# DrQuestion/monica

Measured on AMD Instinct MI355X. Metric: reads/sec classified, higher is better.
Workload: dtype u32/u64 integer; int16 pairs in the alignment kernels (int32 / int8 in the long-call and literal ones); float32 islands: overlap ratio, MAPQ

## Files before the change

monica_amd/csrc/k_fill.hip:

```cpp
#include "device.h"

namespace mnc {

constexpr int FILL_NEG = -(1 << 28);
constexpr int FILL_WIN = 16;
constexpr int FILL_MIN_BAND = 8;
constexpr int FILL_CIG_MAX = 384;
constexpr size_t FILL_P_SLOT = (size_t)(2 * FILL_MAX_LEN + FILL_WIN) * 64;

__device__ __forceinline__ void fill_order()
{
	__builtin_amdgcn_fence(__ATOMIC_SEQ_CST, "wavefront");
	asm volatile("" ::: "memory");
}
__device__ __forceinline__ void fill_order_mem()
{
	__builtin_amdgcn_fence(__ATOMIC_SEQ_CST, "workgroup");
	asm volatile("" ::: "memory");
}

__device__ __forceinline__ int fill_nt4(uint8_t c)
{
	switch (c) {
	case 'A': case 'a': return 0;
	case 'C': case 'c': return 1;
	case 'G': case 'g': return 2;
	case 'T': case 't': case 'U': case 'u': return 3;
	default: return 4;
	}
}

__device__ __forceinline__ int fill_qcode(const Batch &B, bool acgt, int64_t roff, const uint8_t *read, int rlen, int rev, int pq)
{
	const int p = rev ? rlen - 1 - pq : pq;
	if (acgt) {
		const int64_t g = roff + p;
		const int c = (int)(B.packed[g >> 4] >> (30 - 2 * (int)(g & 15)) & 3u);
		return rev ? 3 - c : c;
	}
	const int c = fill_nt4(read[p]);
	return rev ? (c < 4 ? 3 - c : 4) : c;
}

__device__ __forceinline__ uint32_t fill_qcodes16(const Batch &B, int64_t roff, int rlen, int rev, int pq)
{
	int64_t g0 = rev ? roff + rlen - 16 - pq : roff + pq;
	int skip = 0;
	if (g0 < 0) skip = (int)-g0, g0 = 0;
	const uint32_t hi = B.packed[g0 >> 4], lo = B.packed[(g0 >> 4) + 1];
	const uint32_t sh2 = 2 * (uint32_t)(g0 & 15);
	uint32_t f = sh2 ? __builtin_amdgcn_alignbit(hi, lo, 32 - sh2) : hi;
	if (rev) return ~f >> (2 * skip);
	f = __builtin_bitreverse32(f);
	return (f & 0x55555555u) << 1 | (f >> 1 & 0x55555555u);
}

__host__ __device__ __forceinline__ int fill_gap(int l, int q, int e, int q2, int e2)
{
	const int g1 = q + e * l, g2 = q2 + e2 * l;
	return g1 < g2 ? g1 : g2;
}

__host__ __device__ __forceinline__ void fill_band(int n, int m, int cells, int &b, int &kmin, int &kmax)
{
	const int d = n - m, ad = d < 0 ? -d : d;
	b = (2 * cells - 2 - ad) / 2;
	kmin = (d < 0 ? d : 0) - b;
	if (kmin & 1) --kmin;
	kmax = kmin + 2 * cells - 1;
}

__host__ __device__ __forceinline__ int dp_band_bound(int n, int m, int kmin, int kmax, int a, int q, int e, int q2, int e2)
{
	const int d = n - m;
	int U = FILL_NEG;
	{
		const int D0 = kmax + 1, I0 = kmax + 1 - d, left = n - D0;
		if (left >= 0 && m - I0 >= 0) {
			const int u = a * left - fill_gap(D0, q, e, q2, e2) - fill_gap(I0, q, e, q2, e2);
			U = U > u ? U : u;
		}
	}
	{
// ... 189 lines not shown
			fill_order();
		}
		bool walk = leader && ok && !to_next && !to_fb;
		if (walk) {
			int mcols = 0, g2 = 0, kd = 0, kbest = 0;
			for (int k = 0; k < n_c; ++k) {
				const uint32_t op = s_cg[sg][k] & 0xf;
				const int len = (int)(s_cg[sg][k] >> 4);
				if (op == 0) mcols += len, kd = kd - a * len > 0 ? kd - a * len : 0;
				else g2 += fill_gap(len, q, e, q2, e2), kd += q + e * len, kbest = kbest > kd ? kbest : kd;
			}
			const int lost = a * mcols - S - g2;
			const int neg = kbest + lost;
			if (neg <= (B.zdrop_inv < B.zdrop ? B.zdrop_inv : B.zdrop)) walk = false;
		}
		if (walk) {
			int score = 0, mx = INT32_MIN, max_i = -1, max_j = -1, i = 0, j = 0, max_zdrop = 0;
			for (int k = n_c - 1; k >= 0; --k) {
				const uint32_t op = s_cg[sg][k] & 0xf;
				const int len = (int)(s_cg[sg][k] >> 4);
				if (op == 0) {
					for (int l = 0; l < len; ++l) {
						const int ct = s_t[sg][i + l], cq = s_q[sg][j + l];
						score += (ct == 4 || cq == 4) ? scN : ct == cq ? a : bmis;
						if (score < mx) {
							const int li = i + l - max_i, lj = j + l - max_j;
							const int z = mx - score - (li > lj ? li - lj : lj - li) * e;
							max_zdrop = max_zdrop > z ? max_zdrop : z;
						} else mx = score, max_i = i + l, max_j = j + l;
					}
					i += len, j += len;
				} else {
					score -= q + e * len;
					if (op == 1) j += len; else i += len;
					if (score < mx) {
						const int li = i - max_i, lj = j - max_j;
						const int z = mx - score - (li > lj ? li - lj : lj - li) * e;
						max_zdrop = max_zdrop > z ? max_zdrop : z;
					} else mx = score, max_i = i, max_j = j;
				}
			}
			if (max_zdrop > (B.zdrop_inv < B.zdrop ? B.zdrop_inv : B.zdrop)) to_fb = true;
		}
		const bool s_next = __shfl((int)to_next, lead) != 0, s_fb = __shfl((int)to_fb, lead) != 0;
		const int s_nc = __shfl(n_c, lead);
		if (has && (s_next || s_fb)) {
			if (leader) {
				const bool literal = s_fb || next_list == fb_list;
				if (literal && (B.segs[si].flag & SEG_NEEDS_BIG_WS)) { const unsigned long long k = atomicAdd(&B.dp_ctr[56], 1ULL); B.bigfb_list[k] = (int32_t)si; }
				else if (literal) { const unsigned long long k = atomicAdd(&B.dp_ctr[ctr_fb], 1ULL); fb_list[k] = (int32_t)si; }
				else { const unsigned long long k = atomicAdd(&B.dp_ctr[ctr_next], 1ULL); next_list[k] = (int32_t)si; }
			}
		} else if (has) {
			unsigned long long off = 0;
			if (leader) off = atomicAdd(&B.dp_ctr[1], (unsigned long long)s_nc);
			off = (unsigned long long)__shfl((long long)off, lead);
			int wrote = s_nc;
			if ((long long)(off + s_nc) > B.cig_seg_cap) {
				if (leader) atomicMax(&B.dp_ctr[4], 2ULL);
				wrote = 0;
			} else for (int k = L; k < s_nc; k += LANES) B.cig_seg[off + k] = s_cg[sg][s_nc - 1 - k];
			if (leader) {
				Seg *o = B.segs + si;
				o->n_cigar = wrote, o->zdropped = 0, o->zdrop_code = 0;
				o->max = 0, o->max_t = -1, o->max_q = -1, o->score = S, o->reach_end = 0, o->mqe_t = -1;
				o->cig_off = (int64_t)off;
			}
		}
		fill_order_mem();
	}
}

typedef short pk_s16 __attribute__((ext_vector_type(2)));
typedef unsigned short pk_u16 __attribute__((ext_vector_type(2)));
__device__ __forceinline__ uint32_t pk_adds(uint32_t x, uint32_t y) { return __builtin_bit_cast(uint32_t, __builtin_elementwise_add_sat(__builtin_bit_cast(pk_s16, x), __builtin_bit_cast(pk_s16, y))); }
__device__ __forceinline__ uint32_t pk_subs(uint32_t x, uint32_t y) { return __builtin_bit_cast(uint32_t, __builtin_elementwise_sub_sat(__builtin_bit_cast(pk_s16, x), __builtin_bit_cast(pk_s16, y))); }
__device__ __forceinline__ uint32_t pk_maxs(uint32_t x, uint32_t y) { return __builtin_bit_cast(uint32_t, __builtin_elementwise_max(__builtin_bit_cast(pk_s16, x), __builtin_bit_cast(pk_s16, y))); }
__device__ __forceinline__ uint32_t pk_subsu(uint32_t x, uint32_t y) { return __builtin_bit_cast(uint32_t, __builtin_elementwise_sub_sat(__builtin_bit_cast(pk_u16, x), __builtin_bit_cast(pk_u16, y))); }
__device__ __forceinline__ uint32_t pk_madu(uint32_t x, uint32_t y, uint32_t z) { return __builtin_bit_cast(uint32_t, (pk_u16)(__builtin_bit_cast(pk_u16, x) * __builtin_bit_cast(pk_u16, y) + __builtin_bit_cast(pk_u16, z))); }
__device__ __forceinline__ uint32_t pk_rep(int v) { return ((uint32_t)v & 0xffffu) * 0x10001u; }
__device__ __forceinline__ uint32_t pk_bfi(uint32_t mask, uint32_t x, uint32_t y) { return (x & mask) | (y & ~mask); }

constexpr uint32_t PK_NEG = 0x80008000u;
__device__ __forceinline__ uint32_t fillp_opened(uint32_t x)
{
	const uint32_t d = (x & 1u) ^ 1u, c = (x >> 1 & 1u) ^ d, b = (x >> 2 & 1u) ^ 1u ^ c ^ d, a = (x >> 3 & 1u) ^ b ^ c ^ d;
	return a << 3 | b << 2 | c << 1 | d;
}
constexpr uint32_t PK_TAG_H = 0x000f000fu, PK_TAG_E = 0x00070007u, PK_TAG_F = 0x00030003u, PK_TAG_E2 = 0x00010001u;
struct PkConst { uint32_t kmatch, kmis, q8, q28, e8, e28, de28, dstep; int bias; };

__host__ __device__ __forceinline__ bool fillp_bias(int cells, int a, int bmis_abs, int q, int e, int q2, int e2, int &bias)
{
	const int hi = a * FILL_MAX_LEN, lo = -(bmis_abs * FILL_MAX_LEN + fill_gap(2 * cells + 2, q, e, q2, e2) + (q + e > q2 + e2 ? q + e : q2 + e2));
	bias = -(hi + lo) / 2;
	return hi + bias < 2040 && lo + bias > -2040;
}
__host__ __device__ __forceinline__ bool fillp_drifts(int bmis_abs, int e, int e2) { return bmis_abs == 2 * e && e >= e2; }
__host__ __device__ __forceinline__ bool fillp_bias_drift(int a, int q, int e, int q2, int e2, int &bias)
{
	const int hi = (a + 2 * e) * FILL_MAX_LEN, lo = -(q + e + q2 + e2 + 64);
	bias = -(hi + lo) / 2;
	return hi + bias < 2040 && lo + bias > -2040;
}

template <int K> __device__ __forceinline__ uint32_t fillp_next_q(uint32_t Q2, uint32_t w) { return __builtin_amdgcn_perm(Q2, w, 0x05040c00u + K); }
template <int K> __device__ __forceinline__ uint32_t fillp_next_t(uint32_t T2, uint32_t w) { return __builtin_amdgcn_perm(w, T2, 0x0c040302u + K * 0x10000u); }

#ifndef MNC_FILLP_FRAME2
#define MNC_FILLP_FRAME2 1
#endif
template <int LANES, int ODD, bool EDGE, bool CAPTURE = true, bool DRIFT = false, int KB = -1>
__device__ __forceinline__ void fillp_step(const PkConst &K, const int r, const int L, const int rows_m1, const uint8_t *st, const uint8_t *sq,
                                           const int q, const int e, const int q2, const int e2,
                                           int &t_lo, int &tn, int &jn, uint32_t &T2, uint32_t &Q2, uint32_t &Hs,
                                           uint32_t &E, uint32_t &E2, uint32_t &F, uint32_t &F2, uint32_t &Sc,
                                           uint32_t &nb1, uint32_t &nb2, uint32_t &acc, const uint32_t wq = 0, const uint32_t wt = 0)
{
	constexpr int SHR = LANES == 16 ? 0x111 : 0x138, SHL = LANES == 16 ? 0x101 : 0x130;
	constexpr bool SEG_EDGES = LANES != 16 && LANES != 64;
	uint32_t vE, vE2, vF, vF2;
	if (!ODD) {
		nb1 = (uint32_t)__builtin_amdgcn_update_dpp((int)nb1, (int)E, SHR, 0xf, 0xf, false);
		nb2 = (uint32_t)__builtin_amdgcn_update_dpp((int)nb2, (int)E2, SHR, 0xf, 0xf, false);
		if (SEG_EDGES && L == 0) nb1 = nb2 = PK_NEG;
		vE = __builtin_amdgcn_alignbit(E, nb1, 16), vE2 = __builtin_amdgcn_alignbit(E2, nb2, 16);
		vF = F, vF2 = F2;
		if constexpr (KB >= 0) Q2 = fillp_next_q<KB & 3>(Q2, wq);
		else Q2 = __builtin_amdgcn_perm(Q2, (uint32_t)sq[jn], 0x05040100u), ++jn;
	} else {
		nb1 = (uint32_t)__builtin_amdgcn_update_dpp((int)nb1, (int)F, SHL, 0xf, 0xf, false);
		nb2 = (uint32_t)__builtin_amdgcn_update_dpp((int)nb2, (int)F2, SHL, 0xf, 0xf, false);
		if (SEG_EDGES && L == LANES - 1) nb1 = nb2 = PK_NEG;
		vF = __builtin_amdgcn_alignbit(nb1, F, 16), vF2 = __builtin_amdgcn_alignbit(nb2, F2, 16);
		vE = E, vE2 = E2;
		if constexpr (KB >= 0) T2 = fillp_next_t<KB & 3>(T2, wt);
		else T2 = __builtin_amdgcn_perm((uint32_t)st[tn], T2, 0x05040302u), ++tn;
		if (EDGE) ++t_lo;
	}
	uint32_t hd = Hs;
	if (EDGE) {
		const int hb = -fill_gap(r + 1, q, e, q2, e2) + K.bias + (DRIFT ? e * r : 0);
		const uint32_t h0 = pk_rep(((r == 0 ? 0 : -fill_gap(r, q, e, q2, e2)) + K.bias + (DRIFT ? e * (r - 2) : 0)) << 4) | PK_TAG_H;
		const uint32_t g1 = pk_rep((hb - q - e) << 4), g2 = pk_rep((hb - q2 - e2) << 4);
		const uint32_t mt = t_lo == 0 ? 0x0000ffffu : t_lo == -1 ? 0xffff0000u : 0u;
		const uint32_t mj = t_lo == r ? 0x0000ffffu : t_lo == r - 1 ? 0xffff0000u : 0u;
		hd = pk_bfi(mt | mj, h0, hd);
		vE = pk_bfi(mt, g1 | PK_TAG_E, vE), vE2 = pk_bfi(mt, g2 | PK_TAG_E2, vE2);
		vF = pk_bfi(mj, g1 | PK_TAG_F, vF), vF2 = pk_bfi(mj, g2, vF2);
	}
	uint32_t z;
	if (DRIFT) z = pk_madu(pk_subsu(0x00010001u, T2 ^ Q2), K.kmatch, hd);
	else z = pk_adds(hd, pk_madu(pk_subsu(0x00010001u, T2 ^ Q2), K.kmatch, K.kmis));
	uint32_t o2sub = K.q28;
	constexpr bool FRAME2 = DRIFT && MNC_FILLP_FRAME2 && LANES <= 32;
	if (FRAME2) {
		const uint32_t Dr = (uint32_t)r * K.dstep;
		z = pk_maxs(z, vE), z = pk_maxs(z, vF), z = pk_maxs(z, pk_adds(pk_maxs(vE2, vF2), Dr));
		o2sub = K.q28 + Dr;
	} else z = pk_maxs(z, vE), z = pk_maxs(z, vF), z = pk_maxs(z, vE2), z = pk_maxs(z, vF2);
	const uint32_t zt = z | PK_TAG_H;
	const uint32_t o1 = pk_subs(zt, K.q8), o2 = pk_subs(zt, o2sub);
	const uint32_t mE = pk_maxs(vE, o1), mF = pk_maxs(vF, o1), mE2 = pk_maxs(vE2, o2), mF2 = pk_maxs(vF2, o2);
	if (FRAME2) {
		E = mE & 0xfff7fff7u, F = mF & 0xfff3fff3u, E2 = mE2 & 0xfff1fff1u, F2 = mF2 & 0xfff0fff0u;
	} else if (DRIFT) {
		E = mE & 0xfff7fff7u, F = mF & 0xfff3fff3u;
		E2 = pk_adds(mE2, K.de28) & 0xfff1fff1u, F2 = pk_adds(mF2, K.de28) & 0xfff0fff0u;
	} else {
		E = pk_subs(mE, K.e8) & 0xfff7fff7u;
		F = pk_subs(mF, K.e8) & 0xfff3fff3u;
// ... 515 lines not shown
			}
		}
		int bi = -1, bj = -1, reach_end = 0;
		if (ok) {
			if (!zdropped && ez_mqe + B.end_bonus > ez_max) reach_end = 1, bi = ez_mqe_t, bj = m - 1;
			else if (ez_max_t >= 0 && ez_max_q >= 0) bi = ez_max_t, bj = ez_max_q;
		}
		fill_order_mem();
		int state = 0, n_c = 0, wlo = 1 << 30;
		uint32_t cur = 0;
		bool walking = ok && bi >= 0 && bj >= 0, bad = false;
		for (;;) {
			const int seg_r = __shfl(walking ? bi + bj : -1, lead), seg_wlo = __shfl(wlo, lead);
			if (!__any(seg_r >= 0)) break;
			if (seg_r >= 0 && seg_r < seg_wlo) {
				const int lo = seg_r - (FILL_WIN - 1) > 0 ? seg_r - (FILL_WIN - 1) : 0;
#pragma unroll
				for (int k = 0; k < CPL; ++k) {
					const int byte0 = (L + LANES * k) * 16, row = lo + byte0 / W, col = byte0 % W;
					const uint4 v = *reinterpret_cast<const uint4*>(p_wave + (size_t)row * ROWB + lead * CPL + col);
					*reinterpret_cast<uint4*>(&s_win[sg][byte0]) = v;
				}
				wlo = lo;
			}
			fill_order();
			if (leader && walking) {
				while (bi >= 0 && bj >= 0) {
					const int r = bi + bj;
					if (r < wlo) break;
					const int idx = bi - (r - m + 1 > 0 ? r - m + 1 : 0);
					if (idx < 0 || idx >= W) { walking = false, bad = true; break; }
					const uint32_t tmp = s_win[sg][(r - wlo) * W + idx];
					if (state == 0) state = tmp & 7;
					else if (!(tmp >> (state + 2) & 1)) state = 0;
					if (state == 0) state = tmp & 7;
					uint32_t op;
					if (state == 0) op = 0, --bi, --bj;
					else if (state == 1 || state == 3) op = 2, --bi;
					else op = 1, --bj;
					if (cur != 0 && (cur & 0xf) == op) cur += 1u << 4;
					else { if (cur != 0) s_cg[sg][n_c++] = cur; cur = 1u << 4 | op; }
				}
				if (walking && (bi < 0 || bj < 0)) {
					if (bi >= 0) { if (cur != 0 && (cur & 0xf) == 2) cur += (uint32_t)(bi + 1) << 4; else { if (cur != 0) s_cg[sg][n_c++] = cur; cur = (uint32_t)(bi + 1) << 4 | 2; } }
					if (bj >= 0) { if (cur != 0 && (cur & 0xf) == 1) cur += (uint32_t)(bj + 1) << 4; else { if (cur != 0) s_cg[sg][n_c++] = cur; cur = (uint32_t)(bj + 1) << 4 | 1; } }
					if (cur != 0) s_cg[sg][n_c++] = cur;
					walking = false;
				}
			}
			fill_order();
		}
		const bool s_bad = __shfl((int)(bad || (has && !ok)), lead) != 0;
		const int s_nc = __shfl(n_c, lead);
		if (has && s_bad) {
			if (leader && (g.flag & SEG_NEEDS_BIG_WS)) { const unsigned long long k = atomicAdd(&B.dp_ctr[56], 1ULL); B.bigfb_list[k] = (int32_t)si; }
			else if (leader) { const unsigned long long k = atomicAdd(&B.dp_ctr[ctr_fb], 1ULL); fb_list[k] = (int32_t)si; }
		} else if (has) {
			unsigned long long off = 0;
			if (leader && s_nc > 0) off = atomicAdd(&B.dp_ctr[1], (unsigned long long)s_nc);
			off = (unsigned long long)__shfl((long long)off, lead);
			int wrote = s_nc;
			if ((long long)(off + s_nc) > B.cig_seg_cap) {
				if (leader) atomicMax(&B.dp_ctr[4], 2ULL);
				wrote = 0;
			} else {
				const bool keep = (g.flag & EZ_REV_CIGAR) != 0;
				for (int k = L; k < s_nc; k += LANES) B.cig_seg[off + k] = s_cg[sg][keep ? k : s_nc - 1 - k];
			}
			if (leader) {
				Seg *o = B.segs + si;
				o->n_cigar = wrote, o->zdropped = zdropped, o->zdrop_code = 0;
				o->max = ez_max, o->max_t = ez_max_t, o->max_q = ez_max_q, o->score = DP_NEG_INF, o->reach_end = reach_end, o->mqe_t = ez_mqe_t;
				o->cig_off = (int64_t)off;
			}
		}
		fill_order_mem();
	}
}

constexpr int EXTP_G = 16;
constexpr int EXTP_CIG_MAX = 1024;
constexpr int EXTP_ROWS = 2 * FILL_MAX_LEN;

__device__ __forceinline__ uint32_t extp_extended(uint32_t x)
{
	const uint32_t d = x >> 3 & 1u, c = (x >> 2 & 1u) ^ d, b = (x >> 1 & 1u) ^ c ^ d, a = (x & 1u) ^ b ^ c ^ d;
	return d << 3 | c << 2 | b << 1 | a;
}
template <int RGT> struct ExtpTag {
	static constexpr uint32_t H = RGT ? 0u : 0x000f000fu, E = RGT ? 0x00010001u : 0x00070007u, F = 0x00030003u,
	                          E2 = RGT ? 0x00070007u : 0x00010001u, F2 = RGT ? 0x000f000fu : 0u;
};

__host__ __device__ __forceinline__ bool extp_bias(int cells, int a, int bmis_abs, int q, int e, int q2, int e2, int &bias)
{
	const int hi = a * cells, lo = -(bmis_abs * cells + fill_gap(EXTP_ROWS + 32, q, e, q2, e2) + (q + e > q2 + e2 ? q + e : q2 + e2));
	bias = -(hi + lo) / 2;
	return hi + bias < 2040 && lo + bias > -2040 && lo + bias > -2048 + a * cells + 16;
}

template <int LANES, int CPL, int RGT, bool EDGE, bool LIVE>
__device__ __forceinline__ void extp_step(const PkConst &K, const int r, const int L, const int rows, const uint8_t *st, int &tn,
                                          const int q, const int e, const int q2, const int e2, const uint32_t colmask,
                                          uint32_t (&T)[CPL], const uint32_t (&Q)[CPL], uint32_t (&H1)[CPL], uint32_t (&H2)[CPL],
                                          uint32_t (&E)[CPL], uint32_t (&E2)[CPL], uint32_t (&F)[CPL], uint32_t (&F2)[CPL],
                                          uint32_t (&best)[CPL], uint32_t (&bestR)[CPL], uint32_t &nbH, uint32_t &nbF, uint32_t &nbF2,
                                          uint32_t (&acc)[CPL], const int odd)
{
	typedef ExtpTag<RGT> TG;
	constexpr int SHR = LANES == 16 ? 0x111 : 0x138;
	{
		const uint32_t nc = st[tn];
		++tn;
#pragma unroll
		for (int k = CPL - 1; k > 0; --k) T[k] = __builtin_amdgcn_alignbit(T[k], T[k - 1], 16);
		T[0] = __builtin_amdgcn_perm(T[0], nc, 0x05040100u);
	}
	nbH = (uint32_t)__builtin_amdgcn_update_dpp((int)nbH, (int)H2[CPL - 1], SHR, 0xf, 0xf, false);
	nbF = (uint32_t)__builtin_amdgcn_update_dpp((int)nbF, (int)F[CPL - 1], SHR, 0xf, 0xf, false);
	nbF2 = (uint32_t)__builtin_amdgcn_update_dpp((int)nbF2, (int)F2[CPL - 1], SHR, 0xf, 0xf, false);
	uint32_t hd[CPL], vF[CPL], vF2[CPL];
#pragma unroll
	for (int k = CPL - 1; k > 0; --k)
		hd[k] = __builtin_amdgcn_alignbit(H2[k], H2[k - 1], 16), vF[k] = __builtin_amdgcn_alignbit(F[k], F[k - 1], 16), vF2[k] = __builtin_amdgcn_alignbit(F2[k], F2[k - 1], 16);
	hd[0] = __builtin_amdgcn_alignbit(H2[0], nbH, 16), vF[0] = __builtin_amdgcn_alignbit(F[0], nbF, 16), vF2[0] = __builtin_amdgcn_alignbit(F2[0], nbF2, 16);
	const int hb = -fill_gap(r + 1, q, e, q2, e2) + K.bias;
	const uint32_t h0 = pk_rep(((r == 0 ? 0 : -fill_gap(r, q, e, q2, e2)) + K.bias) << 4) | TG::H;
	const uint32_t g1 = pk_rep((hb - q - e) << 4), g2 = pk_rep((hb - q2 - e2) << 4);
	hd[0] = pk_bfi(colmask, h0, hd[0]), vF[0] = pk_bfi(colmask, g1 | TG::F, vF[0]), vF2[0] = pk_bfi(colmask, g2 | TG::F2, vF2[0]);
	uint32_t vE[CPL], vE2[CPL];
#pragma unroll
	for (int k = 0; k < CPL; ++k) vE[k] = E[k], vE2[k] = E2[k];
	if (EDGE) {
		const uint32_t rowmask = L == r / (2 * CPL) ? ((odd & 1) ? 0xffff0000u : 0x0000ffffu) : 0u;
		const int ks = (odd >> 1) % CPL;
#pragma unroll
		for (int k = 0; k < CPL; ++k)
			if (k == ks) hd[k] = pk_bfi(rowmask, h0, hd[k]), vE[k] = pk_bfi(rowmask, g1 | TG::E, vE[k]), vE2[k] = pk_bfi(rowmask, g2 | TG::E2, vE2[k]);
	}
	const uint32_t Rpk = pk_rep(r);
#pragma unroll
	for (int k = 0; k < CPL; ++k) {
		const uint32_t sc = pk_madu(pk_subsu(0x00010001u, T[k] ^ Q[k]), K.kmatch, K.kmis);
		uint32_t z = pk_adds(hd[k], sc);
		z = pk_maxs(z, vE[k]), z = pk_maxs(z, vF[k]), z = pk_maxs(z, vE2[k]), z = pk_maxs(z, vF2[k]);
		const uint32_t zt = RGT ? (z & 0xfff0fff0u) : (z | 0x000f000fu);
		const uint32_t o1 = pk_subs(zt, K.q8), o2 = pk_subs(zt, K.q28);
		const uint32_t mE = pk_maxs(vE[k], o1), mF = pk_maxs(vF[k], o1), mE2 = pk_maxs(vE2[k], o2), mF2 = pk_maxs(vF2[k], o2);
		uint32_t d;
		if (RGT) {
			E[k] = pk_subs(mE, K.e8) | TG::E, F[k] = pk_subs(mF, K.e8) | TG::F, E2[k] = pk_subs(mE2, K.e28) | TG::E2, F2[k] = pk_subs(mF2, K.e28) | TG::F2;
			d = mE ^ mF ^ mE2 ^ mF2;
		} else {
			E[k] = pk_subs(mE, K.e8) & 0xfff7fff7u, F[k] = pk_subs(mF, K.e8) & 0xfff3fff3u, E2[k] = pk_subs(mE2, K.e28) & 0xfff1fff1u, F2[k] = pk_subs(mF2, K.e28) & 0xfff0fff0u;
			d = mE ^ mF ^ mE2 ^ mF2;
		}
		d = pk_bfi(0x000f000fu, z, d << 4);
		acc[k] = (odd & 1) ? __builtin_amdgcn_perm(d, acc[k], 0x06040100u) : __builtin_amdgcn_perm(d, d, 0x0c0c0200u);
		const uint32_t zl = LIVE ? (r < rows ? zt : PK_NEG) : zt;
		const uint32_t nb = pk_maxs(best[k], zl), chg = nb ^ best[k];
		const uint32_t msk = __builtin_bit_cast(uint32_t, (pk_u16)(__builtin_bit_cast(pk_u16, pk_subsu(chg, 0x00010001u)) - __builtin_bit_cast(pk_u16, chg)));
		bestR[k] = pk_bfi(msk, Rpk, bestR[k]), best[k] = nb;
		H2[k] = H1[k], H1[k] = zt;
	}
}

template <int LANES> __device__ __forceinline__ int seg_max_i32(int v)
{
#pragma unroll
	for (int sft = 1; sft < LANES; sft <<= 1) { const int o = __shfl_xor(v, sft); v = v > o ? v : o; }
	return v;
}
template <int LANES> __device__ __forceinline__ unsigned seg_min_u32(unsigned v)
{
#pragma unroll
	for (int sft = 1; sft < LANES; sft <<= 1) { const unsigned o = (unsigned)__shfl_xor((int)v, sft); v = v < o ? v : o; }
	return v;
}
__device__ __forceinline__ int pk_half(uint32_t v, int h) { return (int)(int16_t)(h ? v >> 16 : v & 0xffffu); }

#ifndef MNC_EXTP_WAVES
#define MNC_EXTP_WAVES 4
#endif
template <int LANES, int CPL, int RGT>
__global__ __launch_bounds__(64, MNC_EXTP_WAVES) void mnc_dp_extp(Batch B, const int32_t *list, int ctr_n, int ctr_q, uint8_t *p_all, uint32_t *cig_all)
{
	constexpr int SEGS = 64 / LANES, WC = 2 * CPL * LANES, PAD = WC + 2, SEQ = PAD + EXTP_ROWS + 48;
	constexpr bool LIVE = SEGS > 1;
	constexpr size_t PASS_BYTES = (size_t)FILLP_BLOCKS * 64 * 32 * CPL;
	typedef ExtpTag<RGT> TG;
	__shared__ uint8_t s_t[SEGS][SEQ], s_q[SEGS][WC];
	__shared__ __align__(16) uint8_t s_chunk[64][32];
	__shared__ int32_t s_n[64], s_m[64], s_bi[64], s_bj[64], s_si[64], s_state[64], s_max[64], s_maxt[64], s_maxq[64], s_mqet[64], s_reach[64], s_keep[64];
	const int lane = threadIdx.x, sg = lane / LANES, L = lane % LANES, lead = sg * LANES;
	const bool leader = L == 0;
	const int a = B.sc_a, bmis = -B.sc_b, q = B.gap_q, e = B.gap_e, q2 = B.gap_q2, e2 = B.gap_e2;
	PkConst K;
	K.kmatch = pk_rep((a - bmis) << 4), K.kmis = pk_rep(bmis << 4), K.q8 = pk_rep(q << 4), K.q28 = pk_rep(q2 << 4), K.e8 = pk_rep(e << 4), K.e28 = pk_rep(e2 << 4);
	const bool fits = extp_bias(WC, a, -bmis > B.sc_ambi ? -bmis : B.sc_ambi, q, e, q2, e2, K.bias);
	const int slack = 2 * q + 16 * e + 8 * a + 8 * (-bmis);
	uint8_t *p_wave = p_all + (size_t)blockIdx.x * (EXTP_G * PASS_BYTES);
	uint32_t *cg = cig_all + ((size_t)blockIdx.x * 64 + lane) * EXTP_CIG_MAX;
	const unsigned long long n_items = B.dp_ctr[ctr_n];
	const unsigned long long segmask = LANES == 64 ? ~0ULL : ((1ULL << (LANES & 63)) - 1) << lead;
	const uint32_t colmask = L == 0 ? 0x0000ffffu : 0u;
	int g_eff = (int)((n_items + (unsigned long long)gridDim.x * SEGS - 1) / ((unsigned long long)gridDim.x * SEGS));
	if (g_eff > EXTP_G && g_eff < 2 * EXTP_G) g_eff = (g_eff + 1) / 2;
	g_eff = g_eff < 1 ? 1 : g_eff > EXTP_G ? EXTP_G : g_eff;
	for (;;) {
		unsigned long long q0 = 0;
		if (lane == 0) q0 = atomicAdd(&B.dp_ctr[ctr_q], (unsigned long long)(g_eff * SEGS));
		q0 = (unsigned long long)__shfl((long long)q0, 0);
		if (q0 >= n_items) break;
		s_state[lane] = 0;
		fill_order();
		for (int u = 0; u < g_eff; ++u) {
			if (q0 + (unsigned long long)u * SEGS >= n_items) break;
			const unsigned long long item = q0 + (unsigned long long)u * SEGS + sg;
			const bool has = item < n_items;
			const long long si = has ? (long long)list[item] : -1;
			struct { int32_t tlen, qlen, ts, qs, read, rid, rev, kind, zdrop, flag; } g = { 0, 0, 0, 0, 0, 0, 0, 0, 0, 0 };
			if (has) {
				const Seg *gs = B.segs + si;
				g.tlen = gs->tlen, g.qlen = gs->qlen, g.ts = gs->ts, g.qs = gs->qs, g.read = gs->read, g.rid = gs->rid, g.rev = gs->rev;
				g.kind = gs->kind, g.zdrop = gs->zdrop, g.flag = gs->flag;
			}
			const int n = g.tlen, m = g.qlen;
			bool ok = has && fits && n >= 1 && m >= 1 && m <= WC && n + m - 1 <= EXTP_ROWS && ((g.flag & EZ_RIGHT) != 0) == (RGT != 0);
			const int rows = ok ? n + m - 1 : 0;
			int max_rows = rows, edge_rows = ok ? (m + 15) & ~15 : 0;
#pragma unroll
			for (int sft = LANES; sft < 64; sft <<= 1) {
				const int o = __shfl_xor(max_rows, sft), oe = __shfl_xor(edge_rows, sft);
				max_rows = max_rows > o ? max_rows : o, edge_rows = edge_rows > oe ? edge_rows : oe;
			}
			max_rows = __builtin_amdgcn_readfirstlane(max_rows), edge_rows = __builtin_amdgcn_readfirstlane(edge_rows);
			bool ambiguous = false;
			if (ok) {
				const uint8_t *read = B.bases + B.offsets[g.read];
				const int rlen = (int)(B.offsets[g.read + 1] - B.offsets[g.read]);
				const int64_t coff = B.seq_off[g.rid];
				const bool rv = g.kind == 0;
#pragma unroll 1
				for (int i = L; i < n; i += LANES) {
					const int64_t o = coff + (rv ? g.ts + n - 1 - i : g.ts + i);
					const uint32_t c = B.seq4[o >> 3] >> ((o & 7) * 4) & 15u;
					ambiguous |= c > 3;
					s_t[sg][PAD + i] = (uint8_t)(c & 3);
				}
#pragma unroll 1
				for (int i = n + L; i < max_rows + 16; i += LANES) s_t[sg][PAD + i] = 4;
				const bool acgt = !B.ambig[g.read];
				const int64_t roff = B.offsets[g.read];
#pragma unroll 1
				for (int i = L; i < WC; i += LANES) {
					int c = 5;
					if (i < m) {
						c = fill_qcode(B, acgt, roff, read, rlen, g.rev, rv ? g.qs + m - 1 - i : g.qs + i);
						ambiguous |= c > 3;
						c &= 3;
					}
					s_q[sg][i] = (uint8_t)c;
				}
			}
			const bool seg_amb = (__ballot(ambiguous) & segmask) != 0;
			ok = ok && !seg_amb;
			fill_order();
			const uint8_t *st = &s_t[sg][0];
			uint32_t T[CPL], Q[CPL], H1[CPL], H2[CPL], E[CPL], E2[CPL], F[CPL], F2[CPL], best[CPL], bestR[CPL];
#pragma unroll
			for (int k = 0; k < CPL; ++k) {
				const int c0 = 2 * CPL * L + 2 * k;
				Q[k] = (uint32_t)s_q[sg][c0] | (uint32_t)s_q[sg][c0 + 1] << 16;
				T[k] = (uint32_t)st[PAD - 1 - c0] | (uint32_t)st[PAD - 2 - c0] << 16;
				H1[k] = H2[k] = PK_NEG | TG::H, E[k] = PK_NEG | TG::E, E2[k] = PK_NEG | TG::E2, F[k] = PK_NEG | TG::F, F2[k] = PK_NEG | TG::F2;
				best[k] = PK_NEG | TG::H, bestR[k] = 0;
			}
			int tn = PAD - 2 * CPL * L;
			uint32_t nbH = PK_NEG, nbF = PK_NEG, nbF2 = PK_NEG;
			bool suspect = false;
			uint4 *pblk = reinterpret_cast<uint4*>(p_wave + (size_t)u * PASS_BYTES + (size_t)lane * 32 * CPL);
			for (int r = 0; r < max_rows; r += 16, pblk += 64 * 32 * CPL / 16) {
				uint32_t acc[8][CPL] = {};
				if (r < edge_rows) {
#pragma unroll
					for (int k = 0; k < 16; ++k)
						if (r + k < max_rows) extp_step<LANES, CPL, RGT, true, LIVE>(K, r + k, L, rows, st, tn, q, e, q2, e2, colmask, T, Q, H1, H2, E, E2, F, F2, best, bestR, nbH, nbF, nbF2, acc[k >> 1], k);
				} else {
#pragma unroll
					for (int k = 0; k < 16; ++k)
						if (r + k < max_rows) extp_step<LANES, CPL, RGT, false, LIVE>(K, r + k, L, rows, st, tn, q, e, q2, e2, colmask, T, Q, H1, H2, E, E2, F, F2, best, bestR, nbH, nbF, nbF2, acc[k >> 1], k);
				}
#pragma unroll
				for (int k = 0; k < CPL; ++k)
					pblk[2 * k] = make_uint4(acc[0][k], acc[1][k], acc[2][k], acc[3][k]), pblk[2 * k + 1] = make_uint4(acc[4][k], acc[5][k], acc[6][k], acc[7][k]);
				const int rl = r + 15 < max_rows - 1 ? r + 15 : max_rows - 1;
				int gv = -(1 << 20), av = -(1 << 20);
#pragma unroll
				for (int k = 0; k < CPL; ++k)
#pragma unroll
					for (int h = 0; h < 2; ++h) {
						const int c = 2 * CPL * L + 2 * k + h;
						if (c < m) {
							const int bv = pk_half(best[k], h) >> 4, hv = pk_half(H1[k], h) >> 4;
							gv = gv > bv ? gv : bv;
							if ((unsigned)(rl - c) < (unsigned)n) av = av > hv ? av : hv;
						}
					}
				gv = seg_max_i32<LANES>(gv) - K.bias, av = seg_max_i32<LANES>(av) - K.bias;
				gv = gv > 0 ? gv : 0;
				if (ok && g.zdrop >= 0 && rl < rows && gv - av > g.zdrop - slack) suspect = true;
				bool fin = !ok || !has || r + 16 >= rows;
				{
					const int cm = ok ? m - 1 : 0, src = lead + cm / (2 * CPL), km = cm % (2 * CPL) / 2;
					uint32_t bq = 0;
#pragma unroll
					for (int k = 0; k < CPL; ++k) { const uint32_t x = (uint32_t)__shfl((int)best[k], src); if (k == km) bq = x; }
					int fv = -(1 << 20);
#pragma unroll
					for (int k = 0; k < CPL; ++k) {
						const uint32_t hm = pk_maxs(H1[k], H2[k]);
#pragma unroll
						for (int h = 0; h < 2; ++h) {
							const int c = 2 * CPL * L + 2 * k + h, fc = (pk_half(hm, h) >> 4) + a * (m - 1 - c);
							if (c < m) fv = fv > fc ? fv : fc;
						}
					}
					fv = seg_max_i32<LANES>(fv) - K.bias;
					if (!fin && r + 16 >= m) {
						const int mq = (pk_half(bq, cm & 1) >> 4) - K.bias;
						const int vc = a * m - fill_gap(r + 16, q, e, q2, e2);
						const int bound = fv > vc ? fv : vc;
						const int left = rows - 1 - rl;
#ifdef MNC_EXT_STOP_IGNORES_ZDROP
						const bool no_drop = true;
						(void)left;
#else
						const bool no_drop = g.zdrop < 0 || gv - av + 2 * q2 + e2 * left <= g.zdrop;
#endif
						fin = bound <= gv && bound <= mq && no_drop;
					}
				}
				if (!__any(!fin)) break;
			}
			int ez_max = 0, ez_max_t = -1, ez_max_q = -1, ez_mqe = DP_NEG_INF, ez_mqe_t = -1;
			{
				int gb = -(1 << 20);
#pragma unroll
				for (int k = 0; k < CPL; ++k)
#pragma unroll
					for (int h = 0; h < 2; ++h) { const int bv = pk_half(best[k], h); if (2 * CPL * L + 2 * k + h < m && bv > gb) gb = bv; }
				gb = seg_max_i32<LANES>(gb);
				const int gmax = (gb >> 4) - K.bias;
				if (ok && gmax > 0) {
					unsigned rmin = 0xffffffffu;
#pragma unroll
					for (int k = 0; k < CPL; ++k)
#pragma unroll
						for (int h = 0; h < 2; ++h)
							if (2 * CPL * L + 2 * k + h < m && pk_half(best[k], h) == gb) { const unsigned rr = (h ? bestR[k] >> 16 : bestR[k] & 0xffffu); rmin = rmin < rr ? rmin : rr; }
					rmin = seg_min_u32<LANES>(rmin);
					const int rr = (int)rmin, st0 = rr - m + 1 > 0 ? rr - m + 1 : 0, en0 = rr < n - 1 ? rr : n - 1, en1 = st0 + (en0 - st0) / 4 * 4;
					unsigned key = 0xffffffffu;
#pragma unroll
					for (int k = 0; k < CPL; ++k)
#pragma unroll
						for (int h = 0; h < 2; ++h) {
// ... 35 lines not shown
		const int n = s_n[lane], m = s_m[lane];
		const long long si = s_si[lane];
		int n_c = 0;
		if (state_w == 1) {
			const uint8_t *pu = p_wave + (size_t)(lane / SEGS) * PASS_BYTES;
			const int slot = lane % SEGS;
			int bi = s_bi[lane], bj = s_bj[lane], state = 0, cid = -1;
			uint32_t cur = 0;
			bool walking = bi >= 0 && bj >= 0, bad = false;
			while (walking && bi >= 0 && bj >= 0) {
				const int r = bi + bj;
				const int c = ((r >> 4) * 64 + slot * LANES + bj / (2 * CPL)) * CPL + bj % (2 * CPL) / 2;
				if (c != cid) {
					const uint4 *src = reinterpret_cast<const uint4*>(pu + (size_t)c * 32);
					const uint4 v0 = src[0], v1 = src[1];
					*reinterpret_cast<uint4*>(&s_chunk[lane][0]) = v0, *reinterpret_cast<uint4*>(&s_chunk[lane][16]) = v1;
					cid = c;
				}
				const uint32_t raw = s_chunk[lane][(r & 15) * 2 + (bj & 1)], tag = raw & 15u;
				if (RGT) {
					if (state != 0 && !(extp_extended(raw >> 4) >> (state - 1) & 1u)) state = 0;
					if (state == 0) state = tag == 0u ? 0 : tag == 1u ? 1 : tag == 3u ? 2 : tag == 7u ? 3 : 4;
				} else {
					if (state != 0 && (fillp_opened(raw >> 4) >> (4 - state) & 1u)) state = 0;
					if (state == 0) state = tag >= 8u ? 0 : tag == 7u ? 1 : tag == 3u ? 2 : tag == 1u ? 3 : 4;
				}
				uint32_t op;
				if (state == 0) op = 0, --bi, --bj;
				else if (state == 1 || state == 3) op = 2, --bi;
				else op = 1, --bj;
				if (cur != 0 && (cur & 0xf) == op) cur += 1u << 4;
				else {
					if (cur != 0) {
						if (n_c >= EXTP_CIG_MAX - 4) { bad = true; break; }
						cg[n_c++] = cur;
					}
					cur = 1u << 4 | op;
				}
			}
			if (bad) state_w = 2;
			else if (walking) {
				if (bi >= 0) { if (cur != 0 && (cur & 0xf) == 2) cur += (uint32_t)(bi + 1) << 4; else { if (cur != 0) cg[n_c++] = cur; cur = (uint32_t)(bi + 1) << 4 | 2; } }
				if (bj >= 0) { if (cur != 0 && (cur & 0xf) == 1) cur += (uint32_t)(bj + 1) << 4; else { if (cur != 0) cg[n_c++] = cur; cur = (uint32_t)(bj + 1) << 4 | 1; } }
				if (cur != 0) cg[n_c++] = cur;
			}
		}
		fill_order_mem();
		if (state_w == 2) {
			const int mn = n < m ? n : m;
			const int ci = mn <= 32 ? 16 : mn <= 64 ? 17 : mn <= 128 ? 24 : 25;
			int32_t *lst = mn <= 32 ? B.ext_list1 : mn <= 64 ? B.ext_list2 : mn <= 128 ? B.ext_list3 : B.ext_list4;
			if (mn <= 256) { const unsigned long long k = atomicAdd(&B.dp_ctr[ci], 1ULL); lst[k] = (int32_t)si; }
			else { const unsigned long long k = atomicAdd(&B.dp_ctr[12], 1ULL); B.fill_fb[k] = (int32_t)si; }
		}
		{
			const int mine = state_w == 1 ? n_c : 0;
			int incl = mine;
#pragma unroll
			for (int sft = 1; sft < 64; sft <<= 1) { const int o = __shfl_up(incl, sft); if (lane >= sft) incl += o; }
			const int total = __shfl(incl, 63);
			unsigned long long base = 0;
			if (lane == 0 && total > 0) base = atomicAdd(&B.dp_ctr[1], (unsigned long long)total);
			base = (unsigned long long)__shfl((long long)base, 0);
			const bool over = (long long)(base + total) > B.cig_seg_cap;
			if (over && lane == 0) atomicMax(&B.dp_ctr[4], 2ULL);
			if (state_w == 1) {
				const unsigned long long off = base + (unsigned long long)(incl - mine);
				const bool keep = s_keep[lane] != 0;
				if (!over) for (int k = 0; k < n_c; ++k) B.cig_seg[off + k] = cg[keep ? k : n_c - 1 - k];
				Seg *o = B.segs + si;
				o->n_cigar = over ? 0 : n_c, o->zdropped = 0, o->zdrop_code = 0;
				o->max = s_max[lane], o->max_t = s_maxt[lane], o->max_q = s_maxq[lane], o->score = DP_NEG_INF, o->reach_end = s_reach[lane], o->mqe_t = s_mqet[lane];
				o->cig_off = (int64_t)off;
			}
		}
		fill_order_mem();
	}
}

size_t dp_extp_slot() { return (size_t)EXTP_G * FILLP_BLOCKS * 64 * 32 * 2; }
size_t dp_extp_cig_slot() { return (size_t)64 * EXTP_CIG_MAX * 4; }
void launch_dp_extp(const Batch &B, int cells, int rgt, const int32_t *list, int ctr_n, int ctr_q, uint8_t *p_all, uint32_t *cig_all, int n_wg, hipStream_t st)
{
#define MNC_EXTP(LN, CP) do { if (rgt) hipLaunchKernelGGL((mnc_dp_extp<LN, CP, 1>), dim3(n_wg), dim3(64), 0, st, B, list, ctr_n, ctr_q, p_all, cig_all); \
	else hipLaunchKernelGGL((mnc_dp_extp<LN, CP, 0>), dim3(n_wg), dim3(64), 0, st, B, list, ctr_n, ctr_q, p_all, cig_all); } while (0)
	if (cells == 32) MNC_EXTP(16, 1);
	else if (cells == 64) MNC_EXTP(32, 1);
	else if (cells == 128) MNC_EXTP(64, 1);
	else MNC_EXTP(64, 2);
#undef MNC_EXTP
}

constexpr int LFILL_MAX_LEN = 2047, LFILL_CIG_MAX = 1024;
size_t dp_lfill_p_slot() { return (size_t)(2 * LFILL_MAX_LEN + FILL_WIN) * 64 * 4; }
void launch_dp_lfill(const Batch &B, const int32_t *list, int ctr_n, int ctr_q, int32_t *fb_list, int ctr_fb, uint8_t *p_all, int n_wg, hipStream_t st)
{
	hipLaunchKernelGGL((mnc_dp_fill<64, 4, LFILL_MAX_LEN, LFILL_CIG_MAX>), dim3(n_wg), dim3(64), 0, st, B, list, ctr_n, ctr_q, fb_list, ctr_fb, fb_list, ctr_fb, p_all);
}
constexpr int LEXT_MAX_LEN = 1535;
size_t dp_lext_p_slot() { return (size_t)(2 * LEXT_MAX_LEN + FILL_WIN) * 64 * 8; }
void launch_dp_lext(const Batch &B, const int32_t *list, int ctr_n, int ctr_q, int32_t *fb_list, int ctr_fb, uint8_t *p_all, int n_wg, hipStream_t st)
{
	hipLaunchKernelGGL((mnc_dp_ext<64, 8, LEXT_MAX_LEN>), dim3(n_wg), dim3(64), 0, st, B, list, ctr_n, ctr_q, fb_list, ctr_fb, p_all);
}
size_t dp_fill_p_slot() { return FILL_P_SLOT; }
size_t dp_fillp_slot() { return FILLP_SLOT; }
size_t dp_fillp_cig_slot() { return (size_t)64 * FILL_CIG_MAX * 4; }
void launch_dp_fill(const Batch &B, int lanes, const int32_t *list, int ctr_n, int ctr_q, int32_t *next_list, int ctr_next,
                    int32_t *fb_list, int ctr_fb, uint8_t *p_all, uint32_t *cig_all, int n_wg, hipStream_t st)
{
	bool drift = fillp_drifts(B.sc_b, B.gap_e, B.gap_e2) && !(B.debug_route & 1024);
	if (drift && MNC_FILLP_FRAME2 && lanes <= 64) {
		int bias = 0;
		const bool fits = fillp_bias_drift(B.sc_a, B.gap_q, B.gap_e, B.gap_q2, B.gap_e2, bias);
		const int floor_pts = 2048 + bias;
		const int qmax = B.gap_q > B.gap_q2 ? B.gap_q : B.gap_q2, emax = B.gap_e > B.gap_e2 ? B.gap_e : B.gap_e2;
		const int need = B.sc_a * (lanes + 1) + 2 * qmax + emax * 2 * (lanes + 1) + (B.gap_q2 + B.gap_e2) + 16;
		if (!fits || need >= floor_pts) drift = false;
	}
#define MNC_LAUNCH_FILLP(LN) do { if (drift) hipLaunchKernelGGL((mnc_dp_fillp<LN, true>), dim3(n_wg), dim3(64), 0, st, B, list, ctr_n, ctr_q, next_list, ctr_next, fb_list, ctr_fb, p_all, cig_all); \
	else hipLaunchKernelGGL((mnc_dp_fillp<LN, false>), dim3(n_wg), dim3(64), 0, st, B, list, ctr_n, ctr_q, next_list, ctr_next, fb_list, ctr_fb, p_all, cig_all); } while (0)
	if (lanes == 32) MNC_LAUNCH_FILLP(16);
	else if (lanes == FILL_MID_CELLS) MNC_LAUNCH_FILLP(FILL_MID_CELLS / 2);
	else if (lanes == 64) MNC_LAUNCH_FILLP(32);
	else MNC_LAUNCH_FILLP(64);
#undef MNC_LAUNCH_FILLP
}

void launch_dp_ext(const Batch &B, int lanes, const int32_t *list, int ctr_n, int ctr_q, int32_t *fb_list, int ctr_fb, uint8_t *p_all, int n_wg, hipStream_t st)
{
	if (lanes == 32) hipLaunchKernelGGL((mnc_dp_ext<32, 1, FILL_MAX_LEN>), dim3(n_wg), dim3(64), 0, st, B, list, ctr_n, ctr_q, fb_list, ctr_fb, p_all);
	else if (lanes == 64) hipLaunchKernelGGL((mnc_dp_ext<64, 1, FILL_MAX_LEN>), dim3(n_wg), dim3(64), 0, st, B, list, ctr_n, ctr_q, fb_list, ctr_fb, p_all);
	else if (lanes == 128) hipLaunchKernelGGL((mnc_dp_ext<64, 2, FILL_MAX_LEN>), dim3(n_wg), dim3(64), 0, st, B, list, ctr_n, ctr_q, fb_list, ctr_fb, p_all);
	else hipLaunchKernelGGL((mnc_dp_ext<64, 4, FILL_MAX_LEN>), dim3(n_wg), dim3(64), 0, st, B, list, ctr_n, ctr_q, fb_list, ctr_fb, p_all);
}

}
```

Before: 2.925 million.

## Add lean extension-DP step with word-loaded targets and per-block best tracking

```diff
diff --git a/monica_amd/csrc/extp_dir.h b/monica_amd/csrc/extp_dir.h
--- /dev/null
+++ b/monica_amd/csrc/extp_dir.h
@@ -0,0 +1,38 @@
+#pragma once
+#include <stdint.h>
+
+#if defined(__HIPCC__)
+#define EXTP_FN __host__ __device__ __forceinline__
+#else
+#define EXTP_FN static inline
+#endif
+
+namespace mnc {
+
+template <int RGT> struct ExtpTag {
+	static constexpr uint32_t H = RGT ? 0u : 0x000f000fu, E = RGT ? 0x00010001u : 0x00070007u, F = 0x00030003u,
+	                          E2 = RGT ? 0x00070007u : 0x00010001u, F2 = RGT ? 0x000f000fu : 0u;
+};
+
+EXTP_FN uint32_t fillp_opened(uint32_t x)
+{
+	const uint32_t d = (x & 1u) ^ 1u, c = (x >> 1 & 1u) ^ d, b = (x >> 2 & 1u) ^ 1u ^ c ^ d, a = (x >> 3 & 1u) ^ b ^ c ^ d;
+	return a << 3 | b << 2 | c << 1 | d;
+}
+EXTP_FN uint32_t extp_extended(uint32_t x)
+{
+	const uint32_t d = x >> 3 & 1u, c = (x >> 2 & 1u) ^ d, b = (x >> 1 & 1u) ^ c ^ d, a = (x & 1u) ^ b ^ c ^ d;
+	return d << 3 | c << 2 | b << 1 | a;
+}
+
+EXTP_FN uint32_t extp_dir(uint32_t z, uint32_t mE, uint32_t mF, uint32_t mE2, uint32_t mF2)
+{
+#if defined(__HIP_DEVICE_COMPILE__)
+	const uint32_t x3 = (uint32_t)__builtin_amdgcn_bitop3_b32((int)mE, (int)mF, (int)mE2, 0x96);
+#else
+	const uint32_t x3 = mE ^ mF ^ mE2;
+#endif
+	return (z & 0x000f000fu) | (((x3 ^ mF2) << 4) & ~0x000f000fu);
+}
+
+}
diff --git a/monica_amd/csrc/k_fill.hip b/monica_amd/csrc/k_fill.hip
--- a/monica_amd/csrc/k_fill.hip
+++ b/monica_amd/csrc/k_fill.hip
@@ -1,4 +1,5 @@
 #include "device.h"
+#include "extp_dir.h"
 
 namespace mnc {
 
@@ -354,11 +355,6 @@
 __device__ __forceinline__ uint32_t pk_bfi(uint32_t mask, uint32_t x, uint32_t y) { return (x & mask) | (y & ~mask); }
 
 constexpr uint32_t PK_NEG = 0x80008000u;
-__device__ __forceinline__ uint32_t fillp_opened(uint32_t x)
-{
-	const uint32_t d = (x & 1u) ^ 1u, c = (x >> 1 & 1u) ^ d, b = (x >> 2 & 1u) ^ 1u ^ c ^ d, a = (x >> 3 & 1u) ^ b ^ c ^ d;
-	return a << 3 | b << 2 | c << 1 | d;
-}
 constexpr uint32_t PK_TAG_H = 0x000f000fu, PK_TAG_E = 0x00070007u, PK_TAG_F = 0x00030003u, PK_TAG_E2 = 0x00010001u;
 struct PkConst { uint32_t kmatch, kmis, q8, q28, e8, e28, de28, dstep; int bias; };
 
@@ -1040,15 +1036,6 @@
 constexpr int EXTP_CIG_MAX = 1024;
 constexpr int EXTP_ROWS = 2 * FILL_MAX_LEN;
 
-__device__ __forceinline__ uint32_t extp_extended(uint32_t x)
-{
-	const uint32_t d = x >> 3 & 1u, c = (x >> 2 & 1u) ^ d, b = (x >> 1 & 1u) ^ c ^ d, a = (x & 1u) ^ b ^ c ^ d;
-	return d << 3 | c << 2 | b << 1 | a;
-}
-template <int RGT> struct ExtpTag {
-	static constexpr uint32_t H = RGT ? 0u : 0x000f000fu, E = RGT ? 0x00010001u : 0x00070007u, F = 0x00030003u,
-	                          E2 = RGT ? 0x00070007u : 0x00010001u, F2 = RGT ? 0x000f000fu : 0u;
-};
 
 __host__ __device__ __forceinline__ bool extp_bias(int cells, int a, int bmis_abs, int q, int e, int q2, int e2, int &bias)
 {
@@ -1123,6 +1110,74 @@
 	}
 }
 
+template <int LANES, int CPL, int RGT, bool EDGE, bool LIVE>
+__device__ __forceinline__ void extp_step2(const PkConst &K, const int r, const int L, const int rows, const uint32_t wt,
+                                           const int q, const int e, const int q2, const int e2,
+                                           uint32_t (&T)[CPL], const uint32_t (&Q)[CPL], uint32_t (&H1)[CPL], uint32_t (&H2)[CPL],
+                                           uint32_t (&E)[CPL], uint32_t (&E2)[CPL], uint32_t (&F)[CPL], uint32_t (&F2)[CPL],
+                                           uint32_t (&bb)[CPL], uint32_t &nbH, uint32_t &nbF, uint32_t &nbF2,
+                                           uint32_t (&acc)[CPL], const int odd)
+{
+	typedef ExtpTag<RGT> TG;
+	constexpr int SHR = LANES == 16 ? 0x111 : 0x138;
+	constexpr bool SEG_EDGES = LANES != 16 && LANES != 64;
+#pragma unroll
+	for (int k = CPL - 1; k > 0; --k) T[k] = __builtin_amdgcn_alignbit(T[k], T[k - 1], 16);
+	T[0] = __builtin_amdgcn_perm(T[0], wt, 0x05040c00u + (uint32_t)(odd & 3));
+	const int hb = -fill_gap(r + 1, q, e, q2, e2) + K.bias;
+	const uint32_t h0 = pk_rep(((r == 0 ? 0 : -fill_gap(r, q, e, q2, e2)) + K.bias) << 4) | TG::H;
+	const uint32_t g1 = pk_rep((hb - q - e) << 4), g2 = pk_rep((hb - q2 - e2) << 4);
+	if (!SEG_EDGES) nbH = h0, nbF = g1 | TG::F, nbF2 = g2 | TG::F2;
+	nbH = (uint32_t)__builtin_amdgcn_update_dpp((int)nbH, (int)H2[CPL - 1], SHR, 0xf, 0xf, false);
+	nbF = (uint32_t)__builtin_amdgcn_update_dpp((int)nbF, (int)F[CPL - 1], SHR, 0xf, 0xf, false);
+	nbF2 = (uint32_t)__builtin_amdgcn_update_dpp((int)nbF2, (int)F2[CPL - 1], SHR, 0xf, 0xf, false);
+	if (SEG_EDGES && L == 0) nbH = h0, nbF = g1 | TG::F, nbF2 = g2 | TG::F2;
+	uint32_t hd[CPL], vF[CPL], vF2[CPL];
+#pragma unroll
+	for (int k = CPL - 1; k > 0; --k)
+		hd[k] = __builtin_amdgcn_alignbit(H2[k], H2[k - 1], 16), vF[k] = __builtin_amdgcn_alignbit(F[k], F[k - 1], 16), vF2[k] = __builtin_amdgcn_alignbit(F2[k], F2[k - 1], 16);
+	hd[0] = __builtin_amdgcn_alignbit(H2[0], nbH, 16), vF[0] = __builtin_amdgcn_alignbit(F[0], nbF, 16), vF2[0] = __builtin_amdgcn_alignbit(F2[0], nbF2, 16);
+	uint32_t vE[CPL], vE2[CPL];
+#pragma unroll
+	for (int k = 0; k < CPL; ++k) vE[k] = E[k], vE2[k] = E2[k];
+	if (EDGE) {
+		const uint32_t rowmask = L == r / (2 * CPL) ? ((odd & 1) ? 0xffff0000u : 0x0000ffffu) : 0u;
+		const int ks = (odd >> 1) % CPL;
+#pragma unroll
+		for (int k = 0; k < CPL; ++k)
+			if (k == ks) hd[k] = pk_bfi(rowmask, h0, hd[k]), vE[k] = pk_bfi(rowmask, g1 | TG::E, vE[k]), vE2[k] = pk_bfi(rowmask, g2 | TG::E2, vE2[k]);
+	}
+	const uint32_t kstep = pk_rep(15 - (odd & 15));
+#pragma unroll
+	for (int k = 0; k < CPL; ++k) {
+		const uint32_t sc = pk_madu(pk_subsu(0x00010001u, T[k] ^ Q[k]), K.kmatch, K.kmis);
+		uint32_t z = pk_adds(hd[k], sc);
+		z = pk_maxs(z, vE[k]), z = pk_maxs(z, vF[k]), z = pk_maxs(z, vE2[k]), z = pk_maxs(z, vF2[k]);
+		const uint32_t zt = RGT ? (z & 0xfff0fff0u) : (z | 0x000f000fu);
+		const uint32_t o1 = pk_subs(zt, K.q8), o2 = pk_subs(zt, K.q28);
+		const uint32_t mE = pk_maxs(vE[k], o1), mF = pk_maxs(vF[k], o1), mE2 = pk_maxs(vE2[k], o2), mF2 = pk_maxs(vF2[k], o2);
+		if (RGT) E[k] = pk_subs(mE, K.e8) | TG::E, F[k] = pk_subs(mF, K.e8) | TG::F, E2[k] = pk_subs(mE2, K.e28) | TG::E2, F2[k] = pk_subs(mF2, K.e28) | TG::F2;
+		else E[k] = pk_subs(mE, K.e8) & 0xfff7fff7u, F[k] = pk_subs(mF, K.e8) & 0xfff3fff3u, E2[k] = pk_subs(mE2, K.e28) & 0xfff1fff1u, F2[k] = pk_subs(mF2, K.e28) & 0xfff0fff0u;
+		const uint32_t d = extp_dir(z, mE, mF, mE2, mF2);
+		acc[k] = (odd & 1) ? __builtin_amdgcn_perm(d, acc[k], 0x06040100u) : __builtin_amdgcn_perm(d, d, 0x0c0c0200u);
+		const uint32_t key = (z & 0xfff0fff0u) | kstep;
+		bb[k] = pk_maxs(bb[k], LIVE ? (r < rows ? key : PK_NEG) : key);
+		H2[k] = H1[k], H1[k] = zt;
+	}
+}
+template <int CPL, int RGT>
+__device__ __forceinline__ void extp_block_best(const int r0, const uint32_t (&bb)[CPL], uint32_t (&best)[CPL], uint32_t (&bestR)[CPL])
+{
+	const uint32_t Rpk = pk_rep(r0 + 15);
+#pragma unroll
+	for (int k = 0; k < CPL; ++k) {
+		const uint32_t hs = RGT ? (bb[k] & 0xfff0fff0u) : (bb[k] | 0x000f000fu);
+		const uint32_t nb = pk_maxs(best[k], hs), chg = nb ^ best[k];
+		const uint32_t msk = __builtin_bit_cast(uint32_t, (pk_u16)(__builtin_bit_cast(pk_u16, pk_subsu(chg, 0x00010001u)) - __builtin_bit_cast(pk_u16, chg)));
+		bestR[k] = pk_bfi(msk, Rpk - (bb[k] & 0x000f000fu), bestR[k]), best[k] = nb;
+	}
+}
+
 template <int LANES> __device__ __forceinline__ int seg_max_i32(int v)
 {
 #pragma unroll
@@ -1140,14 +1195,16 @@
 #ifndef MNC_EXTP_WAVES
 #define MNC_EXTP_WAVES 4
 #endif
-template <int LANES, int CPL, int RGT>
+template <int LANES, int CPL, int RGT, bool LEAN>
 __global__ __launch_bounds__(64, MNC_EXTP_WAVES) void mnc_dp_extp(Batch B, const int32_t *list, int ctr_n, int ctr_q, uint8_t *p_all, uint32_t *cig_all)
 {
 	constexpr int SEGS = 64 / LANES, WC = 2 * CPL * LANES, PAD = WC + 2, SEQ = PAD + EXTP_ROWS + 48;
 	constexpr bool LIVE = SEGS > 1;
 	constexpr size_t PASS_BYTES = (size_t)FILLP_BLOCKS * 64 * 32 * CPL;
 	typedef ExtpTag<RGT> TG;
-	__shared__ uint8_t s_t[SEGS][SEQ], s_q[SEGS][WC];
+	static_assert(SEQ % 4 == 0, "extp_step2's target bases are read as words");
+	__shared__ __align__(16) uint8_t s_t[SEGS][SEQ];
+	__shared__ uint8_t s_q[SEGS][WC];
 	__shared__ __align__(16) uint8_t s_chunk[64][32];
 	__shared__ int32_t s_n[64], s_m[64], s_bi[64], s_bj[64], s_si[64], s_state[64], s_max[64], s_maxt[64], s_maxq[64], s_mqet[64], s_reach[64], s_keep[64];
 	const int lane = threadIdx.x, sg = lane / LANES, L = lane % LANES, lead = sg * LANES;
@@ -1240,7 +1297,26 @@
 			uint4 *pblk = reinterpret_cast<uint4*>(p_wave + (size_t)u * PASS_BYTES + (size_t)lane * 32 * CPL);
 			for (int r = 0; r < max_rows; r += 16, pblk += 64 * 32 * CPL / 16) {
 				uint32_t acc[8][CPL] = {};
-				if (r < edge_rows) {
+				if constexpr (LEAN) {
+					const uint32_t *sw = reinterpret_cast<const uint32_t*>(st + (tn & ~3));
+					const uint32_t w0 = sw[0], w1 = sw[1], w2 = sw[2], w3 = sw[3], w4 = sw[4], sh = (uint32_t)(tn & 3) * 8;
+					const uint32_t W[4] = { __builtin_amdgcn_alignbit(w1, w0, sh), __builtin_amdgcn_alignbit(w2, w1, sh),
+					                        __builtin_amdgcn_alignbit(w3, w2, sh), __builtin_amdgcn_alignbit(w4, w3, sh) };
+					tn += 16;
+					uint32_t bb[CPL];
+#pragma unroll
+					for (int k = 0; k < CPL; ++k) bb[k] = PK_NEG;
+					if (r < edge_rows) {
+#pragma unroll
+						for (int k = 0; k < 16; ++k)
+							if (r + k < max_rows) extp_step2<LANES, CPL, RGT, true, LIVE>(K, r + k, L, rows, W[k >> 2], q, e, q2, e2, T, Q, H1, H2, E, E2, F, F2, bb, nbH, nbF, nbF2, acc[k >> 1], k);
+					} else {
+#pragma unroll
+						for (int k = 0; k < 16; ++k)
+							if (r + k < max_rows) extp_step2<LANES, CPL, RGT, false, LIVE>(K, r + k, L, rows, W[k >> 2], q, e, q2, e2, T, Q, H1, H2, E, E2, F, F2, bb, nbH, nbF, nbF2, acc[k >> 1], k);
+					}
+					extp_block_best<CPL, RGT>(r, bb, best, bestR);
+				} else if (r < edge_rows) {
 #pragma unroll
 					for (int k = 0; k < 16; ++k)
 						if (r + k < max_rows) extp_step<LANES, CPL, RGT, true, LIVE>(K, r + k, L, rows, st, tn, q, e, q2, e2, colmask, T, Q, H1, H2, E, E2, F, F2, best, bestR, nbH, nbF, nbF2, acc[k >> 1], k);
@@ -1442,13 +1518,16 @@
 size_t dp_extp_cig_slot() { return (size_t)64 * EXTP_CIG_MAX * 4; }
 void launch_dp_extp(const Batch &B, int cells, int rgt, const int32_t *list, int ctr_n, int ctr_q, uint8_t *p_all, uint32_t *cig_all, int n_wg, hipStream_t st)
 {
-#define MNC_EXTP(LN, CP) do { if (rgt) hipLaunchKernelGGL((mnc_dp_extp<LN, CP, 1>), dim3(n_wg), dim3(64), 0, st, B, list, ctr_n, ctr_q, p_all, cig_all); \
-	else hipLaunchKernelGGL((mnc_dp_extp<LN, CP, 0>), dim3(n_wg), dim3(64), 0, st, B, list, ctr_n, ctr_q, p_all, cig_all); } while (0)
+	const bool lean = !(B.debug_route & 1024);
+#define MNC_EXTP_F(LN, CP, RG, LE) hipLaunchKernelGGL((mnc_dp_extp<LN, CP, RG, LE>), dim3(n_wg), dim3(64), 0, st, B, list, ctr_n, ctr_q, p_all, cig_all)
+#define MNC_EXTP(LN, CP) do { if (rgt) { if (lean) MNC_EXTP_F(LN, CP, 1, true); else MNC_EXTP_F(LN, CP, 1, false); } \
+	else { if (lean) MNC_EXTP_F(LN, CP, 0, true); else MNC_EXTP_F(LN, CP, 0, false); } } while (0)
 	if (cells == 32) MNC_EXTP(16, 1);
 	else if (cells == 64) MNC_EXTP(32, 1);
 	else if (cells == 128) MNC_EXTP(64, 1);
 	else MNC_EXTP(64, 2);
 #undef MNC_EXTP
+#undef MNC_EXTP_F
 }
 
 constexpr int LFILL_MAX_LEN = 2047, LFILL_CIG_MAX = 1024;
```

New measurement: 2.937 million (median of 6 runs). About the same (+0.4%).
